# trinhvg/MoMA

Measured on AMD Instinct MI355X. Metric: images/sec MoMA train step (EffNet-B0 224px, K=65536), higher is better.
Workload: dtype bf16

## Files before the change

### include/moma_hip.h

```cpp
#ifndef MOMA_HIP_H
#define MOMA_HIP_H

#include <stddef.h>
#include <stdint.h>

#ifdef __cplusplus
extern "C" {
#endif

#define MOMA_ABI_VERSION 4

enum { MOMA_PREC_F32 = 0, MOMA_PREC_BF16 = 1 };
enum { MOMA_DT_F32 = 0, MOMA_DT_BF16 = 1 };

enum {
    MOMA_OK = 0,
    MOMA_E_NULL = -1,
    MOMA_E_SHAPE = -2,
    MOMA_E_DTYPE = -3,
    MOMA_E_ALIGN = -4,
    MOMA_E_WORKSPACE = -5,
    MOMA_E_UNSUPPORTED = -6
};

// ... 94 lines not shown
typedef struct moma_mha_module {
    const void* x;
    const void* pack;
    const float* b_qkv;
    const float* b_proj;
    float* y;
    void* qkv16;
    void* attn16;
    float* lse;
    void* qpack;
    float qpack_scale;
    int x_dtype;
} moma_mha_module_t;
size_t moma_mha_pack_bytes(int d);
int moma_mha_pack_weights(const float* w_qkv, const float* w_proj, void* pack, int d, int with_transposed,
                          moma_stream_t stream);
int moma_mha_fwd_fast(const moma_mha_module_t* modules, int n_modules, int N, int d, int H, moma_stream_t stream);
size_t moma_mha_bwd_fast_workspace_bytes(int N, int d, int H);
int moma_mha_bwd_fast(const void* pack, const void* x, int x_dtype, const void* qkv16, const void* attn16, const float* lse,
                      const float* dy, float* dx, float* dw_qkv, float* db_qkv, float* dw_proj, float* db_proj,
                      void* workspace, size_t workspace_bytes, int N, int d, int H, moma_stream_t stream);

enum { MOMA_ACT_NONE = 0, MOMA_ACT_SILU = 1, MOMA_ACT_RELU = 2 };
size_t moma_bn_workspace_bytes(int C);
int moma_bn_fwd(const void* x, void* out, const float* gamma, const float* beta, float* running_mean,
                float* running_var, float* save_mean, float* save_invstd, void* workspace,
                size_t workspace_bytes, int N, int C, int HW, int dtype, int act, int training,
                float momentum, float eps, void* plane_mean, moma_stream_t stream);
int moma_bn_bwd(const void* x, const void* dout, const float* gamma, const float* beta,
                const float* save_mean, const float* save_invstd, void* dx, float* dgamma, float* dbeta,
                void* workspace, size_t workspace_bytes, int N, int C, int HW, int dtype, int act,
                int training, const void* dplane_mean, moma_stream_t stream);

size_t moma_dwconv_workspace_bytes(int C, int K);
int moma_dwconv_fwd(const void* x, const float* w, void* y, int N, int C, int H, int W, int OH, int OW,
                    int K, int stride, int pad_top, int pad_left, int dtype, moma_stream_t stream);
int moma_dwconv_bwd_data(const void* dy, const float* w, void* dx, int N, int C, int H, int W, int OH,
                         int OW, int K, int stride, int pad_top, int pad_left, int dtype,
                         moma_stream_t stream);
int moma_dwconv_bwd_weight(const void* x, const void* dy, float* dw, void* workspace,
                           size_t workspace_bytes, int N, int C, int H, int W, int OH, int OW, int K,
                           int stride, int pad_top, int pad_left, int dtype, moma_stream_t stream);

int moma_plane_mean(const void* x, void* mean, int NC, int HW, int dtype, moma_stream_t stream);
int moma_se_gate_fwd(const void* x, const void* s, void* out, int NC, int HW, int dtype, moma_stream_t stream);
int moma_se_gate_bwd(const void* x, const void* s, const void* dout, void* dx, void* ds, int NC, int HW,
                     int dtype, moma_stream_t stream);

#ifdef __cplusplus
}
#endif
#endif
```

### moma_amd/_lib.py

```python
from __future__ import annotations

import ctypes as C
import os

_HERE = os.path.dirname(os.path.abspath(__file__))
LIB_PATH = os.environ.get("MOMA_HIP_LIB", os.path.join(_HERE, "lib", "libmoma_hip.so"))

PREC_F32, PREC_BF16 = 0, 1
DT_F32, DT_BF16 = 0, 1
LAYOUT_NCHW, LAYOUT_NHWC = 0, 1
MHA_SAVE_PROBS, MHA_SAVE_LSE = 0, 1
ABI_VERSION = 4
EMA_BLOCK_ELEMS = 4096

_p = C.c_void_p
_i = C.c_int
_l = C.c_int64
_f = C.c_float
_z = C.c_size_t

SIGNATURES = {
    "moma_version": (_i, []),
    "moma_error_string": (C.c_char_p, [_i]),
    "moma_debug_set_k2_target_wg": (_i, [_i]),
# ... 10 lines not shown
    "moma_infonce_fused": (_i, [_p, _p, _p, _i, _i, _i, _f, _p, _p, _p, _p, _p, _z, _i, _i, _p]),
    "moma_infonce_fused_ex": (_i, [_p, _p, _p, _i, _i, _i, _f, _p, _p, _p, _p, _p, _z, _i, _i, _p, _p, _p]),
    "moma_infonce_qpack_bytes": (_z, [_i, _i]),
    "moma_infonce_fused_q": (_i, [_p, _p, _p, _p, _i, _i, _i, _f, _p, _p, _p, _p, _p, _z, _i, _i, _p, _p, _p, _p]),
    "moma_infonce_fused_enqueue": (_i, [_p, _p, _p, _p, _i, _i, _i, _f, _p, _p, _p, _p, _p, _z, _i, _i, _p, _i, _l, _p, _p, _p, _p, _p]),
    "moma_infonce_fused_multi_workspace_bytes": (_z, [_i, _i, _i, _i, _i, _i]),
    "moma_infonce_fused_multi": (_i, [_p, _i, _i, _i, _i, _f, _p, _z, _i, _i, _p]),
    "moma_crd_workspace_bytes": (_z, [_i, _i, _i]),
    "moma_crd_fused": (_i, [_p, _p, _p, _p, _p, _i, _i, _i, _l, _f, _p, _i, _p, _p, _p, _p, _p, _z, _p]),
    "moma_crd_scores": (_i, [_p, _p, _p, _p, _p, _i, _i, _i, _l, _f, _p, _i, _p, _p, _p, _p, _z, _p]),
    "moma_crd_scores_bwd": (_i, [_p, _p, _p, _p, _p, _p, _p, _i, _i, _i, _l, _f, _p, _p, _p, _p, _z, _p]),
    "moma_crd_update": (_i, [_p, _p, _p, _p, _p, _i, _i, _l, _f, _p, _p]),
    "moma_at_workspace_bytes": (_z, [_i] * 8),
    "moma_at_map": (_i, [_p, _p] + [_i] * 8 + [_p, _z, _p]),
    "moma_at_pair": (_i, [_p, _p, _i, _i, _p, _p, _p, _p, _p, _p, _p, _p]),
    "moma_at_bwd": (_i, [_p, _p, _p, _p] + [_i] * 8 + [_p]),
    "moma_mha_fwd": (_i,[_p, _p, _p, _p, _p, _p, _p, _p, _p, _i, _i, _i, _i, _p]),
    "moma_mha_saved_state": (_i, [_i, _i, _i, _i]),
    "moma_mha_pack_bytes": (_z, [_i]),
    "moma_mha_pack_weights": (_i, [_p, _p, _p, _i, _i, _p]),
    "moma_mha_fwd_fast": (_i, [_p, _i, _i, _i, _i, _p]),
    "moma_mha_bwd_fast_workspace_bytes": (_z, [_i, _i, _i]),
    "moma_mha_bwd_fast": (_i, [_p, _p, _i, _p, _p, _p, _p, _p, _p, _p, _p, _p, _p, _z, _i, _i, _i, _p]),
    "moma_dwconv_workspace_bytes": (_z, [_i, _i]),
    "moma_dwconv_fwd": (_i, [_p, _p, _p] + [_i] * 11 + [_p]),
    "moma_dwconv_bwd_data": (_i, [_p, _p, _p] + [_i] * 11 + [_p]),
    "moma_dwconv_bwd_weight": (_i, [_p, _p, _p, _p, _z] + [_i] * 11 + [_p]),
    "moma_plane_mean": (_i, [_p, _p, _i, _i, _i, _p]),
    "moma_se_gate_fwd": (_i, [_p, _p, _p, _i, _i, _i, _p]),
    "moma_se_gate_bwd": (_i, [_p, _p, _p, _p, _p, _i, _i, _i, _p]),
    "moma_bn_workspace_bytes": (_z, [_i]),
    "moma_bn_fwd": (_i, [_p, _p, _p, _p, _p, _p, _p, _p, _p, _z, _i, _i, _i, _i, _i, _i, _f, _f, _p, _p]),
    "moma_bn_bwd": (_i, [_p, _p, _p, _p, _p, _p, _p, _p, _p, _p, _z, _i, _i, _i, _i, _i, _i, _p, _p]),
    "moma_mha_bwd_workspace_bytes": (_z, [_i, _i, _i, _i]),
    "moma_mha_bwd": (_i, [_p, _p, _p, _p, _p, _p, _p, _p, _p, _p, _p, _p, _p, _z, _i, _i, _i, _i, _p]),
}



class InfoNCETerm(C.Structure):
    _fields_ = [("q", _p), ("k", _p), ("queue", _p), ("loss_rows", _p), ("lse", _p), ("top1", _p), ("dq", _p)]


class MhaModule(C.Structure):
    _fields_ = [("x", _p), ("pack", _p), ("b_qkv", _p), ("b_proj", _p), ("y", _p), ("qkv16", _p), ("attn16", _p),
                ("lse", _p), ("qpack", _p), ("qpack_scale", _f), ("x_dtype", _i)]


_lib = None


class MomaHipError(RuntimeError):
    pass


def load():
    global _lib
    if _lib is not None:
        return _lib
    import torch
    if not os.path.exists(LIB_PATH):
        raise MomaHipError(
            f"libmoma_hip.so not found at {LIB_PATH}: build it with `python -m moma_amd.build` "
            "(hipcc --offload-arch=gfx950). There is no CPU fallback for the MoMA hot path.")
    lib = C.CDLL(LIB_PATH)
    for name, (res, args) in SIGNATURES.items():
# ... 18 lines not shown
```

### moma_amd/backbones/efficientnet.py

```python
import math
import os

import torch
import torch.nn as nn
import torch.nn.functional as F

_DW_MODE = os.environ.get("MOMA_DW", "hip")
_BN_MODE = os.environ.get("MOMA_BN", "hip")
_SE_MODE = os.environ.get("MOMA_SE", "hip")

_B0_STAGES = [
    (1, 3, 1, 1, 32, 16, 0.25),
    (2, 3, 2, 6, 16, 24, 0.25),
    (2, 5, 2, 6, 24, 40, 0.25),
    (3, 3, 2, 6, 40, 80, 0.25),
    (3, 5, 1, 6, 80, 112, 0.25),
    (4, 5, 2, 6, 112, 192, 0.25),
    (1, 3, 1, 6, 192, 320, 0.25),
]
_BN_MOM, _BN_EPS = 0.01, 1e-3


class _DepthwiseNative(torch.autograd.Function):

# ... 83 lines not shown

    _nbt_pending = 0

    def _flush_nbt(self):
        if self._nbt_pending and self.num_batches_tracked is not None:
            self.num_batches_tracked.add_(self._nbt_pending)
        self._nbt_pending = 0

    def _save_to_state_dict(self, destination, prefix, keep_vars):
        self._flush_nbt()
        super()._save_to_state_dict(destination, prefix, keep_vars)

    def _load_from_state_dict(self, *args, **kwargs):
        self._nbt_pending = 0
        super()._load_from_state_dict(*args, **kwargs)

    def forward(self, x, act=None, want_mean=False):
        if _BN_MODE == "hip" and x.is_cuda and x.dtype in (torch.float32, torch.bfloat16) and self.momentum is not None:
            from .. import ops
            use_batch = self.training or self.running_mean is None
            if self.training and self.track_running_stats and self.num_batches_tracked is not None:
                self._nbt_pending += 1
            return ops.bn_act(x, self.weight, self.bias, self.running_mean, self.running_var, use_batch,
                              self.momentum, self.eps, act, want_mean)
        if _BN_MODE == "aten" and x.is_cuda:
            with torch.backends.cudnn.flags(enabled=False):
                y = super().forward(x)
        else:
            y = super().forward(x)
        y = F.silu(y) if act == "silu" else (F.relu(y) if act == "relu" else y)
        return (y, F.adaptive_avg_pool2d(y, 1)) if want_mean else y


def _drop_connect(x, p, training):
    if not training or not p:
        return x
    keep = 1.0 - p
    mask = torch.floor(keep + torch.rand([x.shape[0], 1, 1, 1], dtype=x.dtype, device=x.device))
    return x / keep * mask


class MBConvBlock(nn.Module):
    def __init__(self, kernel, stride, expand, cin, cout, se_ratio):
        super().__init__()
        mid = cin * expand
        self.expand, self.stride, self.cin, self.cout = expand, stride, cin, cout
        if expand != 1:
            self._expand_conv = SamePadConv2d(cin, mid, 1, bias=False)
            self._bn0 = BatchNorm2d(mid, momentum=_BN_MOM, eps=_BN_EPS)
        self._depthwise_conv = SamePadConv2d(mid, mid, kernel, stride=stride, groups=mid, bias=False)
        self._bn1 = BatchNorm2d(mid, momentum=_BN_MOM, eps=_BN_EPS)
        sq = max(1, int(cin * se_ratio))
        self._se_reduce = SamePadConv2d(mid, sq, 1)
        self._se_expand = SamePadConv2d(sq, mid, 1)
        self._project_conv = SamePadConv2d(mid, cout, 1, bias=False)
        self._bn2 = BatchNorm2d(cout, momentum=_BN_MOM, eps=_BN_EPS)

    def forward(self, x, drop_connect_rate=None):
        inp = x
        if self.expand != 1:
            x = self._bn0(self._expand_conv(x), act="silu")
        x, pooled = self._bn1(self._depthwise_conv(x), act="silu", want_mean=True)
        s = self._se_expand(F.silu(self._se_reduce(pooled)))
        if _SE_MODE == "hip" and x.is_cuda and x.dtype in (torch.float32, torch.bfloat16):
            from .. import ops
            x = ops.se_gate(x, s)
        else:
            x = torch.sigmoid(s) * x
        x = self._bn2(self._project_conv(x))
        if self.stride == 1 and self.cin == self.cout:
            x = _drop_connect(x, drop_connect_rate, self.training) + inp
        return x


class EfficientNet(nn.Module):
    def __init__(self, num_classes=1000, dropout_rate=0.2, drop_connect_rate=0.2, in_channels=3):
        super().__init__()
        self.drop_connect_rate = drop_connect_rate
        self._conv_stem = SamePadConv2d(in_channels, 32, 3, stride=2, bias=False)
        self._bn0 = BatchNorm2d(32, momentum=_BN_MOM, eps=_BN_EPS)
        blocks = []
        for rep, k, s, e, cin, cout, se in _B0_STAGES:
            blocks.append(MBConvBlock(k, s, e, cin, cout, se))
            blocks += [MBConvBlock(k, 1, e, cout, cout, se) for _ in range(rep - 1)]
        self._blocks = nn.ModuleList(blocks)
        self._conv_head = SamePadConv2d(320, 1280, 1, bias=False)
        self._bn1 = BatchNorm2d(1280, momentum=_BN_MOM, eps=_BN_EPS)
        self._avg_pooling = nn.AdaptiveAvgPool2d(1)
        self.classifier_ = nn.Sequential(nn.Dropout(dropout_rate), nn.Linear(1280, num_classes))
        for m in self.modules():
            if isinstance(m, nn.Conv2d):
                nn.init.kaiming_normal_(m.weight, mode="fan_out")
                if m.bias is not None:
                    nn.init.zeros_(m.bias)
            elif isinstance(m, nn.BatchNorm2d):
                nn.init.ones_(m.weight)
                nn.init.zeros_(m.bias)
            elif isinstance(m, nn.Linear):
                nn.init.normal_(m.weight, 0, 0.01)
                nn.init.zeros_(m.bias)

# ... 53 lines not shown
```

### moma_amd/csrc/api.hip

```cpp
#include "common.hpp"

using namespace moma;

namespace {
inline int hip_rc(hipError_t e) { return e == hipSuccess ? MOMA_OK : (int)e; }
inline bool bad_prec(int p) { return p != MOMA_PREC_F32 && p != MOMA_PREC_BF16; }
inline bool bad_dt(int t) { return t != MOMA_DT_F32 && t != MOMA_DT_BF16; }
inline bool misaligned(const void* p, size_t a) { return ((uintptr_t)p % a) != 0; }
inline size_t align_up(size_t x, size_t a) { return (x + a - 1) / a * a; }

#define MOMA_TRY(expr)                         \
    do {                                       \
        hipError_t _e = (expr);                \
        if (_e != hipSuccess) return (int)_e;  \
    } while (0)

GemmArgs gemm(const float* A, const void* B, float* C, int M, int N, int K, long lda, long ldb, long ldc, int tA,
              int tB, float alpha, int prec) {
    GemmArgs g{};
    g.A = A; g.B = B; g.C = C; g.bias = nullptr;
    g.M = M; g.N = N; g.K = K; g.lda = lda; g.ldb = ldb; g.ldc = ldc;
    g.strideA = g.strideB = g.strideC = 0; g.batch = 1;
    g.transA = tA; g.transB = tB; g.alpha = alpha; g.splitk = 1; g.atomic = 0; g.splitC = 0;
    g.b_dtype = MOMA_DT_F32; g.prec = prec;
// ... 415 lines not shown

static int bn_check(int N, int C, int HW, int dtype, int act, const void* ws, size_t ws_bytes) {
    if (N <= 0 || C <= 0 || HW <= 0 || (long)N * C > 0x7fffffffL || (long)N * HW > 0x7fffffffL) return MOMA_E_SHAPE;
    if (dtype != MOMA_DT_F32 && dtype != MOMA_DT_BF16) return MOMA_E_DTYPE;
    if (act != MOMA_ACT_NONE && act != MOMA_ACT_SILU && act != MOMA_ACT_RELU) return MOMA_E_DTYPE;
    if (!ws) return MOMA_E_NULL;
    if (ws_bytes < moma_bn_workspace_bytes(C)) return MOMA_E_WORKSPACE;
    return MOMA_OK;
}

int moma_bn_fwd(const void* x, void* out, const float* gamma, const float* beta, float* running_mean,
                float* running_var, float* save_mean, float* save_invstd, void* workspace, size_t workspace_bytes,
                int N, int C, int HW, int dtype, int act, int training, float momentum, float eps, void* plane_mean,
                moma_stream_t stream) {
    if (!x || !out) return MOMA_E_NULL;
    if (!training && (!running_mean || !running_var)) return MOMA_E_NULL;
    const int rc = bn_check(N, C, HW, dtype, act, workspace, workspace_bytes);
    if (rc != MOMA_OK) return rc;
    return hip_rc(launch_bn_fwd(x, out, gamma, beta, running_mean, running_var, save_mean, save_invstd,
                                (float*)workspace, N, C, HW, dtype, act, training, momentum, eps, plane_mean, (hipStream_t)stream));
}

int moma_bn_bwd(const void* x, const void* dout, const float* gamma, const float* beta, const float* save_mean,
                const float* save_invstd, void* dx, float* dgamma, float* dbeta, void* workspace,
                size_t workspace_bytes, int N, int C, int HW, int dtype, int act, int training,
                const void* dplane_mean, moma_stream_t stream) {
    if (!x || !dout || !save_mean || !save_invstd) return MOMA_E_NULL;
    const int rc = bn_check(N, C, HW, dtype, act, workspace, workspace_bytes);
    if (rc != MOMA_OK) return rc;
    return hip_rc(launch_bn_bwd(x, dout, gamma, beta, save_mean, save_invstd, dx, dgamma, dbeta, (float*)workspace, N,
                                C, HW, dtype, act, training, dplane_mean, (hipStream_t)stream));
}

size_t moma_dwconv_workspace_bytes(int C, int K) {
    return (C > 0 && K > 0) ? align_up(dwconv_workspace_floats(C, K) * sizeof(float), 256) : 0;
}

static int dw_check(int N, int C, int H, int W, int OH, int OW, int K, int S, int pt, int pl, int dtype) {
    if (N <= 0 || C <= 0 || H <= 0 || W <= 0 || OH <= 0 || OW <= 0 || (long)N * C > 0x7fffffffL) return MOMA_E_SHAPE;
    if (!dwconv_supported(K, S)) return MOMA_E_SHAPE;
    if (pt < 0 || pl < 0 || pt >= K || pl >= K) return MOMA_E_SHAPE;
    if ((long)(OH - 1) * S - pt >= H || (long)(OW - 1) * S - pl >= W) return MOMA_E_SHAPE;
    if (dtype != MOMA_DT_F32 && dtype != MOMA_DT_BF16) return MOMA_E_DTYPE;
    return MOMA_OK;
}

int moma_dwconv_fwd(const void* x, const float* w, void* y, int N, int C, int H, int W, int OH, int OW, int K, int stride,
                    int pad_top, int pad_left, int dtype, moma_stream_t stream) {
    if (!x || !w || !y) return MOMA_E_NULL;
    const int rc = dw_check(N, C, H, W, OH, OW, K, stride, pad_top, pad_left, dtype);
    if (rc != MOMA_OK) return rc;
    return hip_rc(launch_dw_fwd(x, w, y, N, C, H, W, OH, OW, K, stride, pad_top, pad_left, dtype, (hipStream_t)stream));
}

int moma_dwconv_bwd_data(const void* dy, const float* w, void* dx, int N, int C, int H, int W, int OH, int OW, int K,
                         int stride, int pad_top, int pad_left, int dtype, moma_stream_t stream) {
    if (!dy || !w || !dx) return MOMA_E_NULL;
    const int rc = dw_check(N, C, H, W, OH, OW, K, stride, pad_top, pad_left, dtype);
    if (rc != MOMA_OK) return rc;
    return hip_rc(launch_dw_bwd_data(dy, w, dx, N, C, H, W, OH, OW, K, stride, pad_top, pad_left, dtype, (hipStream_t)stream));
}

int moma_dwconv_bwd_weight(const void* x, const void* dy, float* dw, void* workspace, size_t workspace_bytes, int N, int C,
                           int H, int W, int OH, int OW, int K, int stride, int pad_top, int pad_left, int dtype,
                           moma_stream_t stream) {
    if (!x || !dy || !dw || !workspace) return MOMA_E_NULL;
// ... 149 lines not shown
```

### moma_amd/csrc/bn.hip

```cpp
#include "common.hpp"

namespace moma {
namespace {

constexpr int BN_THREADS = 256;

template <typename T, int VEC>
struct VecIO;
template <int VEC>
struct VecIO<float, VEC> {
    __device__ static void load(const float* p, float (&v)[VEC]) {
        if constexpr (VEC == 8) {
            const float4 a = *reinterpret_cast<const float4*>(p), b = *reinterpret_cast<const float4*>(p + 4);
            v[0] = a.x; v[1] = a.y; v[2] = a.z; v[3] = a.w; v[4] = b.x; v[5] = b.y; v[6] = b.z; v[7] = b.w;
        } else if constexpr (VEC == 4) {
            const float4 a = *reinterpret_cast<const float4*>(p);
            v[0] = a.x; v[1] = a.y; v[2] = a.z; v[3] = a.w;
        } else {
            v[0] = *p;
        }
    }
    __device__ static void store(float* p, const float (&v)[VEC]) {
        if constexpr (VEC == 8) {
            *reinterpret_cast<float4*>(p) = make_float4(v[0], v[1], v[2], v[3]);
// ... 72 lines not shown
                                                              int N, int C, int HW) {
    const int c = blockIdx.y, s = blockIdx.x, S = gridDim.x;
    const unsigned hwv = HW / VEC, total = (unsigned)N * hwv;
    float sum = 0.f, sq = 0.f, cnt = 0.f;
    for (unsigned i = s * BN_THREADS + threadIdx.x; i < total; i += S * BN_THREADS) {
        const unsigned n = i / hwv, r = i - n * hwv;
        float v[VEC];
        VecIO<T, VEC>::load(x + ((size_t)n * C + c) * HW + (size_t)r * VEC, v);
#pragma unroll
        for (int j = 0; j < VEC; ++j) {
            sum += v[j];
            sq = fmaf(v[j], v[j], sq);
        }
        cnt += (float)VEC;
    }
    float mean = cnt > 0.f ? sum / cnt : 0.f;
    float m2 = fmaxf(sq - sum * mean, 0.f);
#pragma unroll
    for (int o = 32; o > 0; o >>= 1) {
        const float nb = __shfl_xor(cnt, o, 64), mb = __shfl_xor(mean, o, 64), qb = __shfl_xor(m2, o, 64);
        merge(cnt, mean, m2, nb, mb, qb);
    }
    __shared__ float red[BN_THREADS / 64][3];
    const int lane = threadIdx.x & 63, w = threadIdx.x >> 6;
    if (lane == 0) { red[w][0] = cnt; red[w][1] = mean; red[w][2] = m2; }
    __syncthreads();
    if (threadIdx.x == 0) {
        for (int k = 1; k < BN_THREADS / 64; ++k) merge(cnt, mean, m2, red[k][0], red[k][1], red[k][2]);
        float* p = partial + ((size_t)c * S + s) * 3;
        p[0] = cnt; p[1] = mean; p[2] = m2;
    }
}

__global__ __launch_bounds__(256) void bn_finalize_kernel(const float* __restrict__ partial, int S,
                                                          const float* __restrict__ gamma, const float* __restrict__ beta,
                                                          float* __restrict__ running_mean, float* __restrict__ running_var,
                                                          float* __restrict__ save_mean, float* __restrict__ save_invstd,
                                                          float* __restrict__ scale_shift, int C, int training,
                                                          float momentum, float eps) {
    const int lane = threadIdx.x & 63, c = blockIdx.x * 4 + (threadIdx.x >> 6);
    if (c >= C) return;
    float mean, invstd;
    if (training) {
        float n = 0.f, m2 = 0.f;
        mean = 0.f;
        if (lane < S) {
            const float* p = partial + ((size_t)c * S + lane) * 3;
            n = p[0]; mean = p[1]; m2 = p[2];
        }
#pragma unroll
        for (int o = 32; o > 0; o >>= 1) {
            const float nb = __shfl_xor(n, o, 64), mb = __shfl_xor(mean, o, 64), qb = __shfl_xor(m2, o, 64);
            if (lane & o) {
                float n2 = nb, mean2 = mb, m22 = qb;
                merge(n2, mean2, m22, n, mean, m2);
                n = n2; mean = mean2; m2 = m22;
            } else {
                merge(n, mean, m2, nb, mb, qb);
            }
        }
        const float var = m2 / n;
        invstd = rsqrtf(var + eps);
        if (lane == 0) {
            if (running_mean) running_mean[c] = (1.f - momentum) * running_mean[c] + momentum * mean;
            if (running_var) running_var[c] = (1.f - momentum) * running_var[c] + momentum * (n > 1.f ? m2 / (n - 1.f) : var);
        }
    } else {
        mean = running_mean[c];
        invstd = rsqrtf(running_var[c] + eps);
    }
    if (lane == 0) {
        if (save_mean) save_mean[c] = mean;
        if (save_invstd) save_invstd[c] = invstd;
        const float g = gamma ? gamma[c] : 1.f, b = beta ? beta[c] : 0.f;
        scale_shift[2 * c] = g * invstd;
        scale_shift[2 * c + 1] = b - mean * g * invstd;
    }
}

template <typename T, int VEC>
__global__ __launch_bounds__(BN_THREADS) void bn_apply_kernel(const T* __restrict__ x, T* __restrict__ out,
                                                              const float* __restrict__ scale_shift, int C, int HW,
                                                              size_t nvec, int act) {
    const unsigned hwv = HW / VEC;
    for (size_t i = (size_t)blockIdx.x * BN_THREADS + threadIdx.x; i < nvec; i += (size_t)gridDim.x * BN_THREADS) {
        const unsigned plane = (unsigned)(i / hwv), c = plane % (unsigned)C;
        const float sc = scale_shift[2 * c], sh = scale_shift[2 * c + 1];
        float v[VEC];
        VecIO<T, VEC>::load(x + i * VEC, v);
#pragma unroll
        for (int j = 0; j < VEC; ++j) v[j] = act_fwd(fmaf(v[j], sc, sh), act);
        VecIO<T, VEC>::store(out + i * VEC, v);
    }
}

template <typename T, int VEC>
__global__ __launch_bounds__(BN_THREADS) void bn_apply_mean_kernel(const T* __restrict__ x, T* __restrict__ out,
                                                                   T* __restrict__ pmean,
                                                                   const float* __restrict__ scale_shift, int NC, int C,
                                                                   int HW, int act) {
    const int lane = threadIdx.x & 63;
    const int nv = HW / VEC;
    for (int plane = blockIdx.x * (BN_THREADS / 64) + (threadIdx.x >> 6); plane < NC; plane += gridDim.x * (BN_THREADS / 64)) {
        const int c = plane % C;
        const float sc = scale_shift[2 * c], sh = scale_shift[2 * c + 1];
        const T* p = x + (size_t)plane * HW;
        T* o = out + (size_t)plane * HW;
        float acc = 0.f;
        for (int i = lane; i < nv; i += 64) {
            float v[VEC];
            VecIO<T, VEC>::load(p + (size_t)i * VEC, v);
#pragma unroll
            for (int j = 0; j < VEC; ++j) {
                v[j] = act_fwd(fmaf(v[j], sc, sh), act);
                acc += v[j];
            }
            VecIO<T, VEC>::store(o + (size_t)i * VEC, v);
        }
        acc = wave_sum(acc);
        if (lane == 0) {
            float m[1] = {acc / (float)HW};
            VecIO<T, 1>::store(pmean + plane, m);
        }
    }
}

template <typename T, int VEC>
__global__ __launch_bounds__(BN_THREADS) void bn_bwd_reduce_kernel(const T* __restrict__ x, const T* __restrict__ dout,
                                                                   const float* __restrict__ gamma,
                                                                   const float* __restrict__ beta,
                                                                   const float* __restrict__ save_mean,
                                                                   const float* __restrict__ save_invstd,
                                                                   float* __restrict__ partial, int N, int C, int HW,
                                                                   int act, const T* __restrict__ dpl) {
    const int c = blockIdx.y, s = blockIdx.x, S = gridDim.x;
    const unsigned hwv = HW / VEC, total = (unsigned)N * hwv;
    const float mean = save_mean[c], invstd = save_invstd[c];
    const float g = gamma ? gamma[c] : 1.f, b = beta ? beta[c] : 0.f;
    const float inv_hw = 1.f / (float)HW;
    float s1 = 0.f, s2 = 0.f;
    for (unsigned i = s * BN_THREADS + threadIdx.x; i < total; i += S * BN_THREADS) {
        const unsigned n = i / hwv, r = i - n * hwv;
        const size_t off = ((size_t)n * C + c) * HW + (size_t)r * VEC;
        float xv[VEC], dv[VEC];
        VecIO<T, VEC>::load(x + off, xv);
        VecIO<T, VEC>::load(dout + off, dv);
        float add = 0.f;
        if (dpl) { float t1[1]; VecIO<T, 1>::load(dpl + (size_t)n * C + c, t1); add = t1[0] * inv_hw; }
#pragma unroll
        for (int j = 0; j < VEC; ++j) {
            const float xh = (xv[j] - mean) * invstd;
            const float dy = (dv[j] + add) * act_grad(fmaf(xh, g, b), act);
            s1 += dy;
            s2 = fmaf(dy, xh, s2);
        }
// ... 112 lines not shown
        else hipLaunchKernelGGL((bn_apply_mean_kernel<T, 1>), pg, dim3(BN_THREADS), 0, st, x, out, pmean, scale_shift, N * C, C, HW, act);
        return hipGetLastError();
    }
    const unsigned g = apply_grid(nvec);
    if (vec == 8) hipLaunchKernelGGL((bn_apply_kernel<T, 8>), dim3(g), dim3(BN_THREADS), 0, st, x, out, scale_shift, C, HW, nvec, act);
    else if (vec == 4) hipLaunchKernelGGL((bn_apply_kernel<T, 4>), dim3(g), dim3(BN_THREADS), 0, st, x, out, scale_shift, C, HW, nvec, act);
    else hipLaunchKernelGGL((bn_apply_kernel<T, 1>), dim3(g), dim3(BN_THREADS), 0, st, x, out, scale_shift, C, HW, nvec, act);
    return hipGetLastError();
}

template <typename T>
hipError_t bn_bwd_t(const T* x, const T* dout, const float* gamma, const float* beta, const float* save_mean,
                    const float* save_invstd, T* dx, float* dgamma, float* dbeta, float* ws, int N, int C, int HW,
                    int act, int training, const T* dpl, hipStream_t st) {
    const int vec = pick_vec(HW, sizeof(T), x, dout, dx);
    const int S = pick_splits(N, C, HW, vec);
    float* coef = ws;
    float* partial = ws + 3 * (size_t)C;
    const size_t nvec = (size_t)N * C * HW / vec;
    dim3 grid(S, C);
    if (vec == 8) hipLaunchKernelGGL((bn_bwd_reduce_kernel<T, 8>), grid, dim3(BN_THREADS), 0, st, x, dout, gamma, beta, save_mean, save_invstd, partial, N, C, HW, act, dpl);
    else if (vec == 4) hipLaunchKernelGGL((bn_bwd_reduce_kernel<T, 4>), grid, dim3(BN_THREADS), 0, st, x, dout, gamma, beta, save_mean, save_invstd, partial, N, C, HW, act, dpl);
    else hipLaunchKernelGGL((bn_bwd_reduce_kernel<T, 1>), grid, dim3(BN_THREADS), 0, st, x, dout, gamma, beta, save_mean, save_invstd, partial, N, C, HW, act, dpl);
    hipLaunchKernelGGL(bn_bwd_finalize_kernel, dim3((C + 3) / 4), dim3(256), 0, st, partial, S, gamma, save_invstd,
                       dgamma, dbeta, coef, C, (float)N * (float)HW, training);
    if (dx) {
        const unsigned g = apply_grid(nvec);
        if (vec == 8) hipLaunchKernelGGL((bn_bwd_apply_kernel<T, 8>), dim3(g), dim3(BN_THREADS), 0, st, x, dout, dx, gamma, beta, save_mean, save_invstd, coef, C, HW, nvec, act, dpl);
        else if (vec == 4) hipLaunchKernelGGL((bn_bwd_apply_kernel<T, 4>), dim3(g), dim3(BN_THREADS), 0, st, x, dout, dx, gamma, beta, save_mean, save_invstd, coef, C, HW, nvec, act, dpl);
        else hipLaunchKernelGGL((bn_bwd_apply_kernel<T, 1>), dim3(g), dim3(BN_THREADS), 0, st, x, dout, dx, gamma, beta, save_mean, save_invstd, coef, C, HW, nvec, act, dpl);
    }
    return hipGetLastError();
}
}

size_t bn_workspace_floats(int C) { return (size_t)C * (3 + 64 * 3); }

hipError_t launch_bn_fwd(const void* x, void* out, const float* gamma, const float* beta, float* rm, float* rv,
                         float* save_mean, float* save_invstd, float* ws, int N, int C, int HW, int dtype, int act,
                         int training, float momentum, float eps, void* plane_mean, hipStream_t st) {
    if (dtype == MOMA_DT_BF16)
        return bn_fwd_t<bf16_raw>((const bf16_raw*)x, (bf16_raw*)out, gamma, beta, rm, rv, save_mean, save_invstd, ws, N,
                                  C, HW, act, training, momentum, eps, (bf16_raw*)plane_mean, st);
    return bn_fwd_t<float>((const float*)x, (float*)out, gamma, beta, rm, rv, save_mean, save_invstd, ws, N, C, HW, act,
                           training, momentum, eps, (float*)plane_mean, st);
}
hipError_t launch_bn_bwd(const void* x, const void* dout, const float* gamma, const float* beta, const float* save_mean,
                         const float* save_invstd, void* dx, float* dgamma, float* dbeta, float* ws, int N, int C, int HW,
                         int dtype, int act, int training, const void* dplane_mean, hipStream_t st) {
    if (dtype == MOMA_DT_BF16)
        return bn_bwd_t<bf16_raw>((const bf16_raw*)x, (const bf16_raw*)dout, gamma, beta, save_mean, save_invstd,
                                  (bf16_raw*)dx, dgamma, dbeta, ws, N, C, HW, act, training, (const bf16_raw*)dplane_mean, st);
    return bn_bwd_t<float>((const float*)x, (const float*)dout, gamma, beta, save_mean, save_invstd, (float*)dx, dgamma,
                           dbeta, ws, N, C, HW, act, training, (const float*)dplane_mean, st);
}

}
```

### moma_amd/csrc/common.hpp

```cpp
#pragma once
#include <hip/hip_runtime.h>
#include <stdint.h>
#include "../../include/moma_hip.h"

namespace moma {

typedef __attribute__((ext_vector_type(8))) __bf16 bf16x8;
typedef __attribute__((ext_vector_type(4))) __bf16 bf16x4;
typedef __attribute__((ext_vector_type(4))) float f32x4;
typedef __attribute__((ext_vector_type(16))) float f32x16;
typedef unsigned short bf16_raw;

constexpr int WAVE = 64;

__device__ __forceinline__ float bf16_to_f32(bf16_raw v) {
    return __uint_as_float(((unsigned)v) << 16);
}
__device__ __forceinline__ bf16_raw f32_to_bf16(float f) {
    __bf16 b = (__bf16)f;
    return *reinterpret_cast<bf16_raw*>(&b);
}

__device__ __forceinline__ unsigned pack_bf16x2(float lo, float hi) {
    unsigned r;
// ... 157 lines not shown
};
hipError_t launch_infonce_flash(const float* q, const float* k, const void* queue, int B, int d, int K, float inv_T,
                                float* loss_rows, float* lse, int32_t* top1, float* dq, void* ws, int qdtype,
                                hipStream_t st, hipEvent_t ev_begin = nullptr, hipEvent_t ev_end = nullptr,
                                const void* q_packed = nullptr, hipEvent_t ev_call_end = nullptr,
                                const EnqueueJob* enq = nullptr);
size_t infonce_qpack_bytes(int B, int d);
bool infonce_multi_supported(int n_terms, int B, int d, int K, int qdtype, int prec);
size_t infonce_multi_workspace_bytes(int n_terms, int B, int d, int K);
hipError_t launch_infonce_multi(const moma_infonce_term_t* terms, int n_terms, int B, int d, int K, float inv_T, void* ws,
                                hipStream_t st);

bool infonce_f32_flash_supported(int B, int d, int K, int qdtype, int prec);
size_t infonce_f32_flash_workspace_bytes(int B, int d, int K);
hipError_t launch_infonce_f32_flash(const float* q, const float* k, const float* queue, int B, int d, int K, float inv_T,
                                    float* loss_rows, float* lse, int32_t* top1, float* dq, void* ws, hipStream_t st,
                                    hipEvent_t ev_begin = nullptr, hipEvent_t ev_end = nullptr);

bool mha_fast_supported(int N, int d, int H, int prec);
hipError_t launch_mha_pack(const float* w_qkv, const float* w_proj, void* pack, int d, int with_t, hipStream_t st);
hipError_t launch_mha_fwd_fast(const moma_mha_module_t* mods, int n_modules, int N, int d, int H, hipStream_t st);
size_t mha_bwd_fast_workspace_bytes(int N, int d);
hipError_t launch_mha_bwd_fast(const void* pack, const void* x, int x_dtype, const void* qkv16, const void* attn16, const float* lse,
                               const float* dy, float* dx, float* dw_qkv, float* db_qkv, float* dw_proj, float* db_proj,
                               void* workspace, int N, int d, int H, hipStream_t st);

size_t bn_workspace_floats(int C);
hipError_t launch_bn_fwd(const void* x, void* out, const float* gamma, const float* beta, float* rm, float* rv,
                         float* save_mean, float* save_invstd, float* ws, int N, int C, int HW, int dtype, int act,
                         int training, float momentum, float eps, void* plane_mean, hipStream_t st);
hipError_t launch_bn_bwd(const void* x, const void* dout, const float* gamma, const float* beta, const float* save_mean,
                         const float* save_invstd, void* dx, float* dgamma, float* dbeta, float* ws, int N, int C, int HW,
                         int dtype, int act, int training, const void* dplane_mean, hipStream_t st);

bool dwconv_supported(int K, int S);
size_t dwconv_workspace_floats(int C, int K);
hipError_t launch_dw_fwd(const void* x, const float* w, void* y, int N, int C, int H, int W, int OH, int OW, int K, int S,
                         int pt, int pl, int dtype, hipStream_t st);
hipError_t launch_dw_bwd_data(const void* dy, const float* w, void* dx, int N, int C, int H, int W, int OH, int OW, int K,
                              int S, int pt, int pl, int dtype, hipStream_t st);
hipError_t launch_dw_bwd_weight(const void* x, const void* dy, float* dw, float* ws, size_t ws_floats, int N, int C, int H,
                                int W, int OH, int OW, int K, int S, int pt, int pl, int dtype, hipStream_t st);

hipError_t launch_plane_mean(const void* x, void* out, int NC, int HW, int dtype, hipStream_t st);
hipError_t launch_se_gate_fwd(const void* x, const void* s, void* out, int NC, int HW, int dtype, hipStream_t st);
hipError_t launch_se_gate_bwd(const void* x, const void* s, const void* dout, void* dx, void* ds, int NC, int HW, int dtype,
                              hipStream_t st);

}
```

### moma_amd/ops.py

```python
from __future__ import annotations

import ctypes as C
from typing import Sequence, Tuple

import torch

from . import _lib
from ._lib import DT_BF16, DT_F32, PREC_BF16, PREC_F32, EMA_BLOCK_ELEMS, MomaHipError, check

_PREC = {"fp32": PREC_F32, "f32": PREC_F32, "float32": PREC_F32, PREC_F32: PREC_F32,
         "bf16": PREC_BF16, "bfloat16": PREC_BF16, PREC_BF16: PREC_BF16}


def prec_code(p) -> int:
    try:
        return _PREC[p]
    except KeyError:
        raise ValueError(f"unknown precision {p!r}; use 'fp32' or 'bf16'")


def _qdtype(queue: torch.Tensor) -> int:
    if queue.dtype == torch.float32:
        return DT_F32
    if queue.dtype == torch.bfloat16:
# ... 687 lines not shown
        if x.dim() != 4 or x.dtype not in _DT_CODES or s.numel() != x.shape[0] * x.shape[1]:
            raise ValueError(f"se_gate: x {tuple(x.shape)} {x.dtype}, s {tuple(s.shape)}")
        x = x.contiguous()
        s = s.to(x.dtype).contiguous()
        N, Cc, H, W = x.shape
        out = torch.empty_like(x)
        check(lib.moma_se_gate_fwd(_ptr(x), _ptr(s), _ptr(out), N * Cc, H * W, _DT_CODES[x.dtype], _stream()), "moma_se_gate_fwd")
        ctx.save_for_backward(x, s)
        return out

    @staticmethod
    def backward(ctx, dout):
        lib = _lib.load()
        x, s = ctx.saved_tensors
        N, Cc, H, W = x.shape
        dout = dout.contiguous()
        if dout.dtype != x.dtype:
            dout = dout.to(x.dtype)
        dx = torch.empty_like(x)
        ds = torch.empty_like(s)
        check(lib.moma_se_gate_bwd(_ptr(x), _ptr(s), _ptr(dout), _ptr(dx), _ptr(ds), N * Cc, H * W, _DT_CODES[x.dtype],
                                   _stream()), "moma_se_gate_bwd")
        return dx, ds


def plane_mean(x):
    return _PlaneMean.apply(x)


def se_gate(x, s):
    return _SEGate.apply(x, s)


def _crd_check(v1, v2, memory_v1, memory_v2, idx, n_data, Z, bad):
    _dev(v1, "v1"); _dev(v2, "v2"); _dev(memory_v1, "memory_v1"); _dev(memory_v2, "memory_v2")
    _dev(idx, "idx", torch.int64); _dev(Z, "Z"); _dev(bad, "bad_index", torch.int32)
    if (v1.dim() != 2 or v1.shape != v2.shape or memory_v1.dim() != 2 or memory_v1.shape != memory_v2.shape
            or memory_v1.shape[1] != v1.shape[1] or idx.dim() != 2 or idx.shape[0] != v1.shape[0]):
        raise ValueError(f"shape mismatch: v1 {tuple(v1.shape)} v2 {tuple(v2.shape)} memory_v1 {tuple(memory_v1.shape)} "
                         f"memory_v2 {tuple(memory_v2.shape)} idx {tuple(idx.shape)}")
    if int(n_data) != memory_v1.shape[0]:
        raise ValueError(f"n_data {n_data} != rows of the banks {memory_v1.shape[0]}")
    if Z.numel() != 2 or bad.numel() != 1:
        raise ValueError("Z must hold 2 floats (side 1, side 2) and bad_index one int32")


def _crd_workspace(lib, B, d, K1, dev):
    n = lib.moma_crd_workspace_bytes(B, d, K1)
    if n == 0:
        raise MomaHipError(f"moma_crd: unsupported shape B={B} d={d} K1={K1} (d a multiple of 4 up to 2048, nce_k >= 1)")
    return torch.empty(n, device=dev, dtype=torch.uint8), n


class _CRDFused(torch.autograd.Function):

    @staticmethod
    def forward(ctx, v1, v2, memory_v1, memory_v2, idx, T, n_data, Z, set_z, bad):
        lib = _lib.load()
        v1 = v1.contiguous() if isinstance(v1, torch.Tensor) else v1
        v2 = v2.contiguous() if isinstance(v2, torch.Tensor) else v2
        _crd_check(v1, v2, memory_v1, memory_v2, idx, n_data, Z, bad)
        B, d = v1.shape
        K1 = idx.shape[1]
        dev = v1.device
        need_grad = ctx.needs_input_grad[0] or ctx.needs_input_grad[1]
        loss = torch.empty(2, device=dev, dtype=torch.float32)
# ... 187 lines not shown
```

Measured before the change: 6398.

## Fuse BN+SiLU into plane-mean and SE-gate kernels for no-grad MBConv

Adds two kernels for the MBConv tail. The first finalizes BN stats and computes the SiLU-activated plane mean without writing the activated tensor. The second recomputes BN+activation and applies the sigmoid SE gate in one pass. This path is taken only when grad is disabled, so it targets no-grad forwards such as the key/teacher encoder. The aim is to drop one full activation write and read, in exchange for recomputing the BN and SiLU math.

```diff
diff --git a/include/moma_hip.h b/include/moma_hip.h
--- a/include/moma_hip.h
+++ b/include/moma_hip.h
@@ -150,6 +150,13 @@
                 void* workspace, size_t workspace_bytes, int N, int C, int HW, int dtype, int act,
                 int training, const void* dplane_mean, moma_stream_t stream);
 
+int moma_bn_act_plane_mean(const void* x, const float* gamma, const float* beta, float* running_mean,
+                           float* running_var, float* save_mean, float* save_invstd, float* scale_shift,
+                           void* workspace, size_t workspace_bytes, void* plane_mean, int N, int C, int HW,
+                           int dtype, int act, int training, float momentum, float eps, moma_stream_t stream);
+int moma_bn_act_se_gate(const void* x, const float* scale_shift, const void* s, void* out, int N, int C, int HW,
+                        int dtype, int act, moma_stream_t stream);
+
 size_t moma_dwconv_workspace_bytes(int C, int K);
 int moma_dwconv_fwd(const void* x, const float* w, void* y, int N, int C, int H, int W, int OH, int OW,
                     int K, int stride, int pad_top, int pad_left, int dtype, moma_stream_t stream);
diff --git a/moma_amd/_lib.py b/moma_amd/_lib.py
--- a/moma_amd/_lib.py
+++ b/moma_amd/_lib.py
@@ -66,6 +66,8 @@
     "moma_bn_workspace_bytes": (_z, [_i]),
     "moma_bn_fwd": (_i, [_p, _p, _p, _p, _p, _p, _p, _p, _p, _z, _i, _i, _i, _i, _i, _i, _f, _f, _p, _p]),
     "moma_bn_bwd": (_i, [_p, _p, _p, _p, _p, _p, _p, _p, _p, _p, _z, _i, _i, _i, _i, _i, _i, _p, _p]),
+    "moma_bn_act_plane_mean": (_i, [_p, _p, _p, _p, _p, _p, _p, _p, _p, _z, _p, _i, _i, _i, _i, _i, _i, _f, _f, _p]),
+    "moma_bn_act_se_gate": (_i, [_p, _p, _p, _p, _i, _i, _i, _i, _i, _p]),
     "moma_mha_bwd_workspace_bytes": (_z, [_i, _i, _i, _i]),
     "moma_mha_bwd": (_i, [_p, _p, _p, _p, _p, _p, _p, _p, _p, _p, _p, _p, _p, _z, _i, _i, _i, _i, _p]),
 }
diff --git a/moma_amd/backbones/efficientnet.py b/moma_amd/backbones/efficientnet.py
--- a/moma_amd/backbones/efficientnet.py
+++ b/moma_amd/backbones/efficientnet.py
@@ -139,6 +139,18 @@
         return (y, F.adaptive_avg_pool2d(y, 1)) if want_mean else y
 
 
+    def fused_gate_ready(self, x):
+        return _BN_MODE == "hip" and x.is_cuda and x.dtype in (torch.float32, torch.bfloat16) and self.momentum is not None
+
+    def act_plane_mean(self, x, act=None):
+        from .. import ops
+        use_batch = self.training or self.running_mean is None
+        if self.training and self.track_running_stats and self.num_batches_tracked is not None:
+            self._nbt_pending += 1
+        return ops.bn_act_plane_mean(x, self.weight, self.bias, self.running_mean, self.running_var, use_batch,
+                                     self.momentum, self.eps, act)
+
+
 def _drop_connect(x, p, training):
     if not training or not p:
         return x
@@ -167,13 +179,20 @@
         inp = x
         if self.expand != 1:
             x = self._bn0(self._expand_conv(x), act="silu")
-        x, pooled = self._bn1(self._depthwise_conv(x), act="silu", want_mean=True)
-        s = self._se_expand(F.silu(self._se_reduce(pooled)))
-        if _SE_MODE == "hip" and x.is_cuda and x.dtype in (torch.float32, torch.bfloat16):
+        x = self._depthwise_conv(x)
+        if _SE_MODE == "hip" and not torch.is_grad_enabled() and self._bn1.fused_gate_ready(x):
             from .. import ops
-            x = ops.se_gate(x, s)
+            pooled, tail = self._bn1.act_plane_mean(x, act="silu")
+            s = self._se_expand(F.silu(self._se_reduce(pooled)))
+            x = ops.bn_act_se_gate(tail, s)
         else:
-            x = torch.sigmoid(s) * x
+            x, pooled = self._bn1(x, act="silu", want_mean=True)
+            s = self._se_expand(F.silu(self._se_reduce(pooled)))
+            if _SE_MODE == "hip" and x.is_cuda and x.dtype in (torch.float32, torch.bfloat16):
+                from .. import ops
+                x = ops.se_gate(x, s)
+            else:
+                x = torch.sigmoid(s) * x
         x = self._bn2(self._project_conv(x))
         if self.stride == 1 and self.cin == self.cout:
             x = _drop_connect(x, drop_connect_rate, self.training) + inp
diff --git a/moma_amd/csrc/api.hip b/moma_amd/csrc/api.hip
--- a/moma_amd/csrc/api.hip
+++ b/moma_amd/csrc/api.hip
@@ -471,6 +471,32 @@
                                 C, HW, dtype, act, training, dplane_mean, (hipStream_t)stream));
 }
 
+int moma_bn_act_plane_mean(const void* x, const float* gamma, const float* beta, float* running_mean, float* running_var,
+                           float* save_mean, float* save_invstd, float* scale_shift, void* workspace, size_t workspace_bytes,
+                           void* plane_mean, int N, int C, int HW, int dtype, int act, int training, float momentum, float eps,
+                           moma_stream_t stream) {
+    if (!x || !scale_shift || !plane_mean) return MOMA_E_NULL;
+    if (!training && (!running_mean || !running_var)) return MOMA_E_NULL;
+    const int rc = bn_check(N, C, HW, dtype, act, workspace, workspace_bytes);
+    if (rc != MOMA_OK) return rc;
+    return hip_rc(launch_bn_act_plane_mean(x, gamma, beta, running_mean, running_var, save_mean, save_invstd, scale_shift,
+                                           (float*)workspace, plane_mean, N, C, HW, dtype, act, training, momentum, eps,
+                                           (hipStream_t)stream));
+}
+
+static int tail_check(int N, int C, int HW, int dtype, int act) {
+    if (N <= 0 || C <= 0 || HW <= 0 || (long)N * C > 0x7fffffffL) return MOMA_E_SHAPE;
+    if (dtype != MOMA_DT_F32 && dtype != MOMA_DT_BF16) return MOMA_E_DTYPE;
+    if (act != MOMA_ACT_NONE && act != MOMA_ACT_SILU && act != MOMA_ACT_RELU) return MOMA_E_DTYPE;
+    return MOMA_OK;
+}
+int moma_bn_act_se_gate(const void* x, const float* scale_shift, const void* s, void* out, int N, int C, int HW, int dtype,
+                        int act, moma_stream_t stream) {
+    if (!x || !scale_shift || !s || !out) return MOMA_E_NULL;
+    const int rc = tail_check(N, C, HW, dtype, act);
+    return rc != MOMA_OK ? rc : hip_rc(launch_bn_act_se_gate(x, scale_shift, s, out, N, C, HW, dtype, act, (hipStream_t)stream));
+}
+
 size_t moma_dwconv_workspace_bytes(int C, int K) {
     return (C > 0 && K > 0) ? align_up(dwconv_workspace_floats(C, K) * sizeof(float), 256) : 0;
 }
diff --git a/moma_amd/csrc/bn.hip b/moma_amd/csrc/bn.hip
--- a/moma_amd/csrc/bn.hip
+++ b/moma_amd/csrc/bn.hip
@@ -128,14 +128,16 @@
     }
 }
 
-__global__ __launch_bounds__(256) void bn_finalize_kernel(const float* __restrict__ partial, int S,
-                                                          const float* __restrict__ gamma, const float* __restrict__ beta,
-                                                          float* __restrict__ running_mean, float* __restrict__ running_var,
-                                                          float* __restrict__ save_mean, float* __restrict__ save_invstd,
-                                                          float* __restrict__ scale_shift, int C, int training,
-                                                          float momentum, float eps) {
-    const int lane = threadIdx.x & 63, c = blockIdx.x * 4 + (threadIdx.x >> 6);
-    if (c >= C) return;
+template <typename T> __device__ __forceinline__ float round_to(float v);
+template <> __device__ __forceinline__ float round_to<float>(float v) { return v; }
+template <> __device__ __forceinline__ float round_to<bf16_raw>(float v) { return bf16_to_f32(f32_to_bf16(v)); }
+
+__device__ __forceinline__ void bn_channel_finalize(const float* __restrict__ partial, int S, const float* __restrict__ gamma,
+                                                    const float* __restrict__ beta, float* __restrict__ running_mean,
+                                                    float* __restrict__ running_var, float* __restrict__ save_mean,
+                                                    float* __restrict__ save_invstd, float* __restrict__ scale_shift, int c,
+                                                    int lane, int training, float momentum, float eps, bool write, float& sc,
+                                                    float& sh) {
     float mean, invstd;
     if (training) {
         float n = 0.f, m2 = 0.f;
@@ -157,7 +159,7 @@
         }
         const float var = m2 / n;
         invstd = rsqrtf(var + eps);
-        if (lane == 0) {
+        if (write && lane == 0) {
             if (running_mean) running_mean[c] = (1.f - momentum) * running_mean[c] + momentum * mean;
             if (running_var) running_var[c] = (1.f - momentum) * running_var[c] + momentum * (n > 1.f ? m2 / (n - 1.f) : var);
         }
@@ -165,13 +167,28 @@
         mean = running_mean[c];
         invstd = rsqrtf(running_var[c] + eps);
     }
-    if (lane == 0) {
+    const float g = gamma ? gamma[c] : 1.f, b = beta ? beta[c] : 0.f;
+    sc = g * invstd;
+    sh = b - mean * g * invstd;
+    if (write && lane == 0) {
         if (save_mean) save_mean[c] = mean;
         if (save_invstd) save_invstd[c] = invstd;
-        const float g = gamma ? gamma[c] : 1.f, b = beta ? beta[c] : 0.f;
-        scale_shift[2 * c] = g * invstd;
-        scale_shift[2 * c + 1] = b - mean * g * invstd;
-    }
+        scale_shift[2 * c] = sc;
+        scale_shift[2 * c + 1] = sh;
+    }
+}
+
+__global__ __launch_bounds__(256) void bn_finalize_kernel(const float* __restrict__ partial, int S,
+                                                          const float* __restrict__ gamma, const float* __restrict__ beta,
+                                                          float* __restrict__ running_mean, float* __restrict__ running_var,
+                                                          float* __restrict__ save_mean, float* __restrict__ save_invstd,
+                                                          float* __restrict__ scale_shift, int C, int training,
+                                                          float momentum, float eps) {
+    const int lane = threadIdx.x & 63, c = blockIdx.x * 4 + (threadIdx.x >> 6);
+    if (c >= C) return;
+    float sc, sh;
+    bn_channel_finalize(partial, S, gamma, beta, running_mean, running_var, save_mean, save_invstd, scale_shift, c, lane,
+                        training, momentum, eps, true, sc, sh);
 }
 
 template <typename T, int VEC>
@@ -217,6 +234,66 @@
         if (lane == 0) {
             float m[1] = {acc / (float)HW};
             VecIO<T, 1>::store(pmean + plane, m);
+        }
+    }
+}
+
+template <typename T, int VEC>
+__global__ __launch_bounds__(BN_THREADS) void bn_act_plane_mean_kernel(const T* __restrict__ x, T* __restrict__ pmean,
+                                                                       const float* __restrict__ partial, int S,
+                                                                       const float* __restrict__ gamma,
+                                                                       const float* __restrict__ beta,
+                                                                       float* __restrict__ running_mean,
+                                                                       float* __restrict__ running_var,
+                                                                       float* __restrict__ save_mean,
+                                                                       float* __restrict__ save_invstd,
+                                                                       float* __restrict__ scale_shift, int NC, int C, int HW,
+                                                                       int act, int training, float momentum, float eps) {
+    const int lane = threadIdx.x & 63;
+    const int nv = HW / VEC;
+    for (int plane = blockIdx.x * (BN_THREADS / 64) + (threadIdx.x >> 6); plane < NC; plane += gridDim.x * (BN_THREADS / 64)) {
+        const int c = plane % C;
+        float sc, sh;
+        bn_channel_finalize(partial, S, gamma, beta, running_mean, running_var, save_mean, save_invstd, scale_shift, c, lane,
+                            training, momentum, eps, plane < C, sc, sh);
+        const T* p = x + (size_t)plane * HW;
+        float acc = 0.f;
+        for (int i = lane; i < nv; i += 64) {
+            float v[VEC];
+            VecIO<T, VEC>::load(p + (size_t)i * VEC, v);
+#pragma unroll
+            for (int j = 0; j < VEC; ++j) {
+                v[j] = act_fwd(fmaf(v[j], sc, sh), act);
+                acc += v[j];
+            }
+        }
+        acc = wave_sum(acc);
+        if (lane == 0) {
+            float m[1] = {acc / (float)HW};
+            VecIO<T, 1>::store(pmean + plane, m);
+        }
+    }
+}
+
+template <typename T, int VEC>
+__global__ __launch_bounds__(BN_THREADS) void bn_act_se_gate_kernel(const T* __restrict__ x, const T* __restrict__ s,
+                                                                    T* __restrict__ out,
+                                                                    const float* __restrict__ scale_shift, int NC, int C,
+                                                                    int HW, int act) {
+    const int lane = threadIdx.x & 63;
+    const int nv = HW / VEC;
+    for (int plane = blockIdx.x * (BN_THREADS / 64) + (threadIdx.x >> 6); plane < NC; plane += gridDim.x * (BN_THREADS / 64)) {
+        const int c = plane % C;
+        const float sc = scale_shift[2 * c], sh = scale_shift[2 * c + 1];
+        const float g = 1.f / (1.f + __expf(-ld1<T>(s + plane)));
+        const T* p = x + (size_t)plane * HW;
+        T* o = out + (size_t)plane * HW;
+        for (int i = lane; i < nv; i += 64) {
+            float v[VEC];
+            VecIO<T, VEC>::load(p + (size_t)i * VEC, v);
+#pragma unroll
+            for (int j = 0; j < VEC; ++j) v[j] = round_to<T>(act_fwd(fmaf(v[j], sc, sh), act)) * g;
+            VecIO<T, VEC>::store(o + (size_t)i * VEC, v);
         }
     }
 }
@@ -395,6 +472,41 @@
     }
     return hipGetLastError();
 }
+unsigned plane_grid(int NC) {
+    long gp = ((long)NC + BN_THREADS / 64 - 1) / (BN_THREADS / 64);
+    if (gp > 256 * 32) gp = 256 * 32;
+    return (unsigned)(gp < 1 ? 1 : gp);
+}
+template <typename T>
+hipError_t bn_act_plane_mean_t(const T* x, const float* gamma, const float* beta, float* rm, float* rv, float* save_mean,
+                               float* save_invstd, float* scale_shift, float* partial, T* pmean, int N, int C, int HW, int act,
+                               int training, float momentum, float eps, hipStream_t st) {
+    const int vec = pick_vec(HW, sizeof(T), x, nullptr, nullptr);
+    const int S = training ? pick_splits(N, C, HW, vec) : 1;
+    if (training) {
+        dim3 grid(S, C);
+        if (vec == 8) hipLaunchKernelGGL((bn_stats_kernel<T, 8>), grid, dim3(BN_THREADS), 0, st, x, partial, N, C, HW);
+        else if (vec == 4) hipLaunchKernelGGL((bn_stats_kernel<T, 4>), grid, dim3(BN_THREADS), 0, st, x, partial, N, C, HW);
+        else hipLaunchKernelGGL((bn_stats_kernel<T, 1>), grid, dim3(BN_THREADS), 0, st, x, partial, N, C, HW);
+    }
+    const dim3 pg(plane_grid(N * C));
+    if (vec == 8) hipLaunchKernelGGL((bn_act_plane_mean_kernel<T, 8>), pg, dim3(BN_THREADS), 0, st, x, pmean, partial, S, gamma, beta, rm, rv, save_mean, save_invstd, scale_shift, N * C, C, HW, act, training, momentum, eps);
+    else if (vec == 4) hipLaunchKernelGGL((bn_act_plane_mean_kernel<T, 4>), pg, dim3(BN_THREADS), 0, st, x, pmean, partial, S, gamma, beta, rm, rv, save_mean, save_invstd, scale_shift, N * C, C, HW, act, training, momentum, eps);
+    else hipLaunchKernelGGL((bn_act_plane_mean_kernel<T, 1>), pg, dim3(BN_THREADS), 0, st, x, pmean, partial, S, gamma, beta, rm, rv, save_mean, save_invstd, scale_shift, N * C, C, HW, act, training, momentum, eps);
+    return hipGetLastError();
+}
+
+template <typename T>
+hipError_t bn_act_se_gate_t(const T* x, const float* scale_shift, const T* s, T* out, int N, int C, int HW, int act,
+                            hipStream_t st) {
+    const int vec = pick_vec(HW, sizeof(T), x, out, nullptr);
+    const dim3 pg(plane_grid(N * C));
+    if (vec == 8) hipLaunchKernelGGL((bn_act_se_gate_kernel<T, 8>), pg, dim3(BN_THREADS), 0, st, x, s, out, scale_shift, N * C, C, HW, act);
+    else if (vec == 4) hipLaunchKernelGGL((bn_act_se_gate_kernel<T, 4>), pg, dim3(BN_THREADS), 0, st, x, s, out, scale_shift, N * C, C, HW, act);
+    else hipLaunchKernelGGL((bn_act_se_gate_kernel<T, 1>), pg, dim3(BN_THREADS), 0, st, x, s, out, scale_shift, N * C, C, HW, act);
+    return hipGetLastError();
+}
+
 }
 
 size_t bn_workspace_floats(int C) { return (size_t)C * (3 + 64 * 3); }
@@ -418,4 +530,22 @@
                            dbeta, ws, N, C, HW, act, training, (const float*)dplane_mean, st);
 }
 
-}
+hipError_t launch_bn_act_plane_mean(const void* x, const float* gamma, const float* beta, float* rm, float* rv,
+                                    float* save_mean, float* save_invstd, float* scale_shift, float* ws, void* plane_mean,
+                                    int N, int C, int HW, int dtype, int act, int training, float momentum, float eps,
+                                    hipStream_t st) {
+    float* partial = ws + 2 * (size_t)C;
+    if (dtype == MOMA_DT_BF16)
+        return bn_act_plane_mean_t<bf16_raw>((const bf16_raw*)x, gamma, beta, rm, rv, save_mean, save_invstd, scale_shift,
+                                             partial, (bf16_raw*)plane_mean, N, C, HW, act, training, momentum, eps, st);
+    return bn_act_plane_mean_t<float>((const float*)x, gamma, beta, rm, rv, save_mean, save_invstd, scale_shift, partial,
+                                      (float*)plane_mean, N, C, HW, act, training, momentum, eps, st);
+}
+hipError_t launch_bn_act_se_gate(const void* x, const float* scale_shift, const void* s, void* out, int N, int C, int HW,
+                                 int dtype, int act, hipStream_t st) {
+    if (dtype == MOMA_DT_BF16)
+        return bn_act_se_gate_t<bf16_raw>((const bf16_raw*)x, scale_shift, (const bf16_raw*)s, (bf16_raw*)out, N, C, HW, act, st);
+    return bn_act_se_gate_t<float>((const float*)x, scale_shift, (const float*)s, (float*)out, N, C, HW, act, st);
+}
+
+}
diff --git a/moma_amd/csrc/common.hpp b/moma_amd/csrc/common.hpp
--- a/moma_amd/csrc/common.hpp
+++ b/moma_amd/csrc/common.hpp
@@ -213,6 +213,12 @@
 hipError_t launch_bn_bwd(const void* x, const void* dout, const float* gamma, const float* beta, const float* save_mean,
                          const float* save_invstd, void* dx, float* dgamma, float* dbeta, float* ws, int N, int C, int HW,
                          int dtype, int act, int training, const void* dplane_mean, hipStream_t st);
+hipError_t launch_bn_act_plane_mean(const void* x, const float* gamma, const float* beta, float* rm, float* rv,
+                                    float* save_mean, float* save_invstd, float* scale_shift, float* ws, void* plane_mean,
+                                    int N, int C, int HW, int dtype, int act, int training, float momentum, float eps,
+                                    hipStream_t st);
+hipError_t launch_bn_act_se_gate(const void* x, const float* scale_shift, const void* s, void* out, int N, int C, int HW,
+                                 int dtype, int act, hipStream_t st);
 
 bool dwconv_supported(int K, int S);
 size_t dwconv_workspace_floats(int C, int K);
diff --git a/moma_amd/ops.py b/moma_amd/ops.py
--- a/moma_amd/ops.py
+++ b/moma_amd/ops.py
@@ -743,6 +743,55 @@
     return _SEGate.apply(x, s)
 
 
+class BNGateState:
+    __slots__ = ("x", "scale_shift", "cfg")
+
+    def __init__(self, x, scale_shift, cfg):
+        self.x, self.scale_shift, self.cfg = x, scale_shift, cfg
+
+
+def _no_grad_only(name, *tensors):
+    if torch.is_grad_enabled() and any(t is not None and t.requires_grad for t in tensors):
+        raise MomaHipError(f"{name}: forward only -- no backward kernels exist for the fused MBConv tail; "
+                           "use bn_act(..., want_mean=True) and se_gate where a gradient is recorded")
+
+
+def bn_act_plane_mean(x, weight, bias, running_mean, running_var, training: bool, momentum: float, eps: float, act=None):
+    lib = _lib.load()
+    _dev(x, "x", dtype=None, contiguous=False)
+    if x.dim() != 4 or x.dtype not in _DT_CODES:
+        raise ValueError(f"bn_act_plane_mean: expects [N,C,H,W] float32 / bfloat16, got {tuple(x.shape)} {x.dtype}")
+    _no_grad_only("bn_act_plane_mean", x, weight, bias)
+    x = x.detach().contiguous()
+    N, Cc = x.shape[0], x.shape[1]
+    HW = x.shape[2] * x.shape[3]
+    dev = x.device
+    scale_shift = torch.empty(Cc, 2, device=dev, dtype=torch.float32)
+    ws = torch.empty(lib.moma_bn_workspace_bytes(Cc), device=dev, dtype=torch.uint8)
+    pmean = torch.empty(N, Cc, 1, 1, device=dev, dtype=x.dtype)
+    act = ACT_CODES[act]
+    check(lib.moma_bn_act_plane_mean(_ptr(x), _ptr(weight), _ptr(bias), _ptr(running_mean), _ptr(running_var), _ptr(None),
+                                     _ptr(None), _ptr(scale_shift), _ptr(ws), ws.numel(), _ptr(pmean), N, Cc, HW,
+                                     _DT_CODES[x.dtype], act, int(bool(training)), float(momentum), float(eps), _stream()),
+          "moma_bn_act_plane_mean")
+    return pmean, BNGateState(x, scale_shift, (N, Cc, HW, act))
+
+
+def bn_act_se_gate(state: BNGateState, s):
+    lib = _lib.load()
+    x = state.x
+    N, Cc, HW, act = state.cfg
+    _dev(s, "s", dtype=None, contiguous=False)
+    if s.numel() != N * Cc:
+        raise ValueError(f"bn_act_se_gate: x {tuple(x.shape)} {x.dtype}, s {tuple(s.shape)}")
+    _no_grad_only("bn_act_se_gate", s)
+    s = s.detach().to(x.dtype).contiguous()
+    out = torch.empty_like(x)
+    check(lib.moma_bn_act_se_gate(_ptr(x), _ptr(state.scale_shift), _ptr(s), _ptr(out), N, Cc, HW, _DT_CODES[x.dtype], act,
+                                  _stream()), "moma_bn_act_se_gate")
+    return out
+
+
 def _crd_check(v1, v2, memory_v1, memory_v2, idx, n_data, Z, bad):
     _dev(v1, "v1"); _dev(v2, "v2"); _dev(memory_v1, "memory_v1"); _dev(memory_v2, "memory_v2")
     _dev(idx, "idx", torch.int64); _dev(Z, "Z"); _dev(bad, "bad_index", torch.int32)
```

After: 6195. 0.968x the previous value.
